# siyaoL1/Analytical-Database

Hardware: AMD Instinct MI355X
Metric: rows/sec scanned + HBM GB/s (% of roofline), 1B-row int32 select+sum (higher is better)
Workload: dtype int32; 1 GPU; 1B-row single int32 column, range select + sum; rows_per_gpu=1000000000, low=250000000, high=260000000, parallelism=single GPU

## Files before the change

### analytical-database_amd/csrc/mq_kernels.hip

```cpp

#include <hip/hip_runtime.h>

#include <atomic>
#include <condition_variable>
#include <mutex>
#include <thread>
#include <vector>
#include <climits>
#include <cstdarg>
#include <cstdint>
#include <cstdio>
#include <cstdlib>
#include <cstring>

#include <cerrno>
#include <pthread.h>
#include <sched.h>
#include <sys/mman.h>

#ifndef MADV_POPULATE_WRITE
#define MADV_POPULATE_WRITE 23
#endif

#include "mq_common.h"
#include "mq_device.h"
#include "mq_scan_common.h"

__device__ int mq_writelane(int src, int lane, int old) __asm("llvm.amdgcn.writelane.i32");

namespace {

using namespace mqi;

__device__ __forceinline__ void store_agent(unsigned long long* p, unsigned long long v) {
    __hip_atomic_store(p, v, __ATOMIC_RELAXED, __HIP_MEMORY_SCOPE_AGENT);
}
__device__ __forceinline__ unsigned long long load_agent(const unsigned long long* p) {
    return __hip_atomic_load(const_cast<unsigned long long*>(p), __ATOMIC_RELAXED,
                             __HIP_MEMORY_SCOPE_AGENT);
}

template <bool WT = false>
__device__ __forceinline__ void block_store_partial(unsigned long long cnt, long long sum, int mn,
                                                    int mx, Partial* __restrict__ part) {
    __shared__ Partial sp[kWaves];
    const int lane = threadIdx.x & 63, wave = threadIdx.x >> 6;
    cnt = wave_sum_u64(cnt);
    sum = wave_sum_i64(sum);
    mn = wave_min(mn);
    mx = wave_max(mx);
    if (lane == 0) sp[wave] = Partial{cnt, sum, mn, mx, 0ull};
    __syncthreads();
    if (threadIdx.x == 0) {
        Partial r = sp[0];
#pragma unroll
        for (int w = 1; w < kWaves; w++) {
            r.count += sp[w].count;
            r.sum += sp[w].sum;
            r.mn = min(r.mn, sp[w].mn);
            r.mx = max(r.mx, sp[w].mx);
        }
        if constexpr (WT) {
            unsigned long long* w = reinterpret_cast<unsigned long long*>(part + blockIdx.x);
            store_agent(w + 0, r.count);
            store_agent(w + 1, (unsigned long long)r.sum);
            store_agent(w + 2, (unsigned long long)(uint32_t)r.mn | ((unsigned long long)(uint32_t)r.mx << 32));
        } else {
            part[blockIdx.x] = r;
        }
    }
}

constexpr int kArriveStride = 1024;
constexpr size_t kArriveBytes = 9 * kArriveStride * sizeof(unsigned int);

__device__ __forceinline__ bool block_arrive_last(uint32_t nblocks, unsigned int* ctr) {
    __shared__ int s_last;
    if (threadIdx.x == 0) {
        const uint32_t shard = blockIdx.x & 7u;
        const uint32_t shard_n = (nblocks - shard + 7u) / 8u;
        __builtin_amdgcn_s_waitcnt(0x0F70);
        int last = 0;
        if (__hip_atomic_fetch_add(ctr + shard * kArriveStride, 1u, __ATOMIC_RELAXED,
                                   __HIP_MEMORY_SCOPE_AGENT) == shard_n - 1u) {
            const uint32_t nshards = nblocks < 8u ? nblocks : 8u;
            last = __hip_atomic_fetch_add(ctr + 8 * kArriveStride, 1u, __ATOMIC_RELAXED,
                                          __HIP_MEMORY_SCOPE_AGENT) == nshards - 1u;
        }
        if (last) {
#pragma unroll
            for (int i = 0; i < 9; i++)
                __hip_atomic_store(ctr + i * kArriveStride, 0u, __ATOMIC_RELAXED,
                                   __HIP_MEMORY_SCOPE_AGENT);
        }
        s_last = last;
    }
    __syncthreads();
    return s_last != 0;
}

__device__ __forceinline__ void block_combine(const Partial* __restrict__ part, uint32_t nparts,
                                              mq_agg* __restrict__ out) {
    unsigned long long cnt = 0;
    long long sum = 0;
    int mn = INT_MAX, mx = INT_MIN;
    for (uint32_t base = 0; base < nparts; base += 8 * blockDim.x) {
        unsigned long long c[8], sm[8], m[8];
#pragma unroll
        for (int j = 0; j < 8; j++) {
            const uint32_t i = base + j * blockDim.x + threadIdx.x;
            const unsigned long long* w =
                reinterpret_cast<const unsigned long long*>(part + (i < nparts ? i : nparts - 1));
            c[j] = load_agent(w + 0);
            sm[j] = load_agent(w + 1);
            m[j] = load_agent(w + 2);
        }
#pragma unroll
        for (int j = 0; j < 8; j++) {
            if (base + j * blockDim.x + threadIdx.x >= nparts) {
                c[j] = 0ull;
                sm[j] = 0ull;
                m[j] = 0x800000007FFFFFFFull;
            }
        }
#pragma unroll
        for (int j = 0; j < 8; j++) {
            cnt += c[j];
            sum += (long long)sm[j];
            mn = min(mn, (int)(uint32_t)m[j]);
            mx = max(mx, (int)(uint32_t)(m[j] >> 32));
        }
    }
    __shared__ Partial sc[kWaves];
    const int lane = threadIdx.x & 63, wave = threadIdx.x >> 6;
    cnt = wave_sum_u64(cnt);
    sum = wave_sum_i64(sum);
    mn = wave_min(mn);
    mx = wave_max(mx);
    if (lane == 0) sc[wave] = Partial{cnt, sum, mn, mx, 0ull};
    __syncthreads();
    if (threadIdx.x == 0) {
        Partial r = sc[0];
#pragma unroll
        for (int w = 1; w < kWaves; w++) {
            r.count += sc[w].count;
            r.sum += sc[w].sum;
            r.mn = min(r.mn, sc[w].mn);
            r.mx = max(r.mx, sc[w].mx);
        }
        out->count = r.count;
        out->sum = r.sum;
        out->min = r.mn;
        out->max = r.mx;
        out->_pad = 0;
    }
}

enum ScanMode { kSum = 0, kAgg = 1 };

template <int MODE>
struct ScanTraits {
    static constexpr int kUnrollM = MODE == kAgg ? 6 : kUnroll;
};

template <int MODE, bool VEC>
__global__ __launch_bounds__(kTPB, 8) void k_scan(const int* __restrict__ col, uint64_t n,
                                               uint64_t rows_per_block, Pred pred,
                                               Partial* __restrict__ part,
                                               mq_agg* __restrict__ out, unsigned int* __restrict__ arrive) {
    const uint64_t start = (uint64_t)blockIdx.x * rows_per_block;
    uint64_t end = start + rows_per_block;
    if (end > n) end = n;
    const int tid = threadIdx.x;
    const uint32_t lo = pred.lo, wm1 = pred.wm1;

    unsigned int cnt = 0;
    unsigned long long sumd = 0;
    uint32_t mind = 0xFFFFFFFFu;
    uint32_t maxr = 0xFFFFFFFFu;

    auto consume = [&](int4 v, uint64_t tile_row, bool full) {
        const uint64_t row = tile_row + (uint64_t)tid * 4;
        const uint32_t d0 = (uint32_t)v.x - lo, d1 = (uint32_t)v.y - lo, d2 = (uint32_t)v.z - lo,
                       d3 = (uint32_t)v.w - lo;
        bool p0 = d0 <= wm1, p1 = d1 <= wm1, p2 = d2 <= wm1, p3 = d3 <= wm1;
        if (!full) {
            p0 = p0 && (row + 0 < end);
            p1 = p1 && (row + 1 < end);
            p2 = p2 && (row + 2 < end);
            p3 = p3 && (row + 3 < end);
        }
        cnt += (unsigned)p0 + (unsigned)p1 + (unsigned)p2 + (unsigned)p3;
        sumd += (unsigned long long)(p0 ? d0 : 0u) + (unsigned long long)(p1 ? d1 : 0u) +
                (unsigned long long)(p2 ? d2 : 0u) + (unsigned long long)(p3 ? d3 : 0u);
        if constexpr (MODE == kAgg) {
            if (full) {
                mind = min(mind, min(min(d0, d1), min(d2, d3)));
                maxr = min(maxr, min(min(wm1 - d0, wm1 - d1), min(wm1 - d2, wm1 - d3)));
            } else {
                mind = min(mind, min(min(p0 ? d0 : ~0u, p1 ? d1 : ~0u), min(p2 ? d2 : ~0u, p3 ? d3 : ~0u)));
                maxr = min(maxr, min(min(p0 ? wm1 - d0 : ~0u, p1 ? wm1 - d1 : ~0u),
                                     min(p2 ? wm1 - d2 : ~0u, p3 ? wm1 - d3 : ~0u)));
            }
        }
    };

    constexpr int U = ScanTraits<MODE>::kUnrollM;
    uint64_t t = start;
    for (; t + (uint64_t)U * kTileRows <= end; t += (uint64_t)U * kTileRows) {
        int4 v[U];
#pragma unroll
        for (int u = 0; u < U; u++)
            v[u] = load4_nt<VEC>(col + t + (uint64_t)u * kTileRows + (uint64_t)tid * 4);
#pragma unroll
        for (int u = 0; u < U; u++) consume(v[u], t + (uint64_t)u * kTileRows, true);
    }
    for (; t < end; t += kTileRows) {
        const uint64_t row = t + (uint64_t)tid * 4;
        int4 v;
        if (row + 3 < end) {
            v = load4_nt<VEC>(col + row);
        } else {
            v.x = row + 0 < end ? col[row + 0] : 0;
            v.y = row + 1 < end ? col[row + 1] : 0;
            v.z = row + 2 < end ? col[row + 2] : 0;
            v.w = row + 3 < end ? col[row + 3] : 0;
        }
        consume(v, t, row + 3 < end);
    }
    const long long sum = (long long)sumd + (long long)cnt * (long long)(int32_t)lo;
    int mn = INT_MAX, mx = INT_MIN;
    if (MODE == kAgg && cnt) {
        mn = (int)(lo + mind);
        mx = (int)(lo + (wm1 - maxr));
    }
    if (out) {
        block_store_partial<true>(cnt, sum, mn, mx, part);
        if (block_arrive_last(gridDim.x, arrive)) block_combine(part, gridDim.x, out);
    } else {
        block_store_partial(cnt, sum, mn, mx, part);
    }
}

template <bool VEC>
__global__ __launch_bounds__(kTPB, 8) void k_stream_read(const int* __restrict__ col, uint64_t n,
                                                         uint64_t rows_per_block,
                                                         uint32_t* __restrict__ out) {
    const uint64_t start = (uint64_t)blockIdx.x * rows_per_block;
    uint64_t end = start + rows_per_block;
    if (end > n) end = n;
    const int tid = threadIdx.x;
    uint32_t x = 0;
    for (uint64_t t = start; t + 8ull * kTileRows <= end; t += 8ull * kTileRows) {
        int4 v[8];
#pragma unroll
        for (int u = 0; u < 8; u++)
            v[u] = load4_nt<VEC>(col + t + (uint64_t)u * kTileRows + (uint64_t)tid * 4);
#pragma unroll
        for (int u = 0; u < 8; u++) x ^= (uint32_t)(v[u].x ^ v[u].y ^ v[u].z ^ v[u].w);
    }
    x = (uint32_t)wave_sum_u64(x);
    if ((tid & 63) == 0) atomicXor(out + blockIdx.x, x);
}

__global__ __launch_bounds__(kTPB) void k_final(const Partial* __restrict__ part, uint32_t nparts,
                                                mq_agg* __restrict__ out) {
    unsigned long long cnt = 0;
    long long sum = 0;
    int mn = INT_MAX, mx = INT_MIN;
    for (uint32_t i = threadIdx.x; i < nparts; i += kTPB) {
        const Partial p = part[i];
        cnt += p.count;
        sum += p.sum;
        mn = min(mn, p.mn);
        mx = max(mx, p.mx);
    }
    __shared__ Partial sp[kWaves];
    const int lane = threadIdx.x & 63, wave = threadIdx.x >> 6;
    cnt = wave_sum_u64(cnt);
    sum = wave_sum_i64(sum);
    mn = wave_min(mn);
    mx = wave_max(mx);
    if (lane == 0) sp[wave] = Partial{cnt, sum, mn, mx, 0ull};
    __syncthreads();
    if (threadIdx.x == 0) {
        Partial r = sp[0];
        for (int w = 1; w < kWaves; w++) {
            r.count += sp[w].count;
            r.sum += sp[w].sum;
            r.mn = min(r.mn, sp[w].mn);
            r.mx = max(r.mx, sp[w].mx);
        }
        out->count = r.count;
        out->sum = r.sum;
        out->min = r.mn;
        out->max = r.mx;
        out->_pad = 0;
    }
}

constexpr int kStTiles = 8;
constexpr int kStGranule = 256 * kStTiles;
constexpr int kStBuf = 1024;
constexpr unsigned long long kStDone = 1ull << 63;

__device__ __forceinline__ uint32_t rank_lt(unsigned long long m, uint32_t acc) {
    return __builtin_amdgcn_mbcnt_hi((uint32_t)(m >> 32), __builtin_amdgcn_mbcnt_lo((uint32_t)m, acc));
}

struct StageState {
    uint32_t fill;
    uint32_t flushed;
    uint32_t nbm;
    uint64_t sw;
    bool bmode;
};

template <bool PAYLOAD, int BUF, bool FULL, int J>
__device__ __forceinline__ void stage_tile(StageState& st, int4 v, uint32_t t0, uint32_t E, uint32_t lo,
                                           uint32_t wm1, int32_t base, int lane, int* buf,
                                           const int* __restrict__ payload,
                                           unsigned long long* __restrict__ bm, int* __restrict__ spill,
                                           uint32_t r0, int& rlo, int& rhi) {
    const uint32_t row0 = t0 + (uint32_t)lane * 4;
    bool p0 = ((uint32_t)v.x - lo) <= wm1, p1 = ((uint32_t)v.y - lo) <= wm1,
         p2 = ((uint32_t)v.z - lo) <= wm1, p3 = ((uint32_t)v.w - lo) <= wm1;
    if (!FULL) {
        p0 = p0 && row0 + 0 < E;
        p1 = p1 && row0 + 1 < E;
        p2 = p2 && row0 + 2 < E;
        p3 = p3 && row0 + 3 < E;
    }
    const unsigned long long m0 = __ballot(p0), m1 = __ballot(p1), m2 = __ballot(p2),
                             m3 = __ballot(p3);
    const uint32_t c = __builtin_amdgcn_readfirstlane(
        (uint32_t)(__popcll(m0) + __popcll(m1) + __popcll(m2) + __popcll(m3)));
    if (!st.bmode) {
        if (c == 0) return;
        const uint32_t over = st.fill + c - st.flushed;
        const uint32_t need = __builtin_amdgcn_readfirstlane(
            over > (uint32_t)BUF ? ((over - (uint32_t)BUF + 63u) & ~63u) : 0u);
        if (st.flushed + need <= 8u * r0) {
            if (need) {
                __builtin_amdgcn_wave_barrier();
                for (uint32_t f = 0; f < need; f += 64u) {
                    const uint32_t i = st.flushed + f + (uint32_t)lane;
                    spill[i] = buf[i % (uint32_t)BUF];
                }
                st.flushed = __builtin_amdgcn_readfirstlane(st.flushed + need);
            }
            uint32_t k = rank_lt(m3, rank_lt(m2, rank_lt(m1, rank_lt(m0, st.fill))));
            if (p0) buf[(k++) % (uint32_t)BUF] = PAYLOAD ? payload[row0 + 0] : (int)(row0 + 0) + base;
            if (p1) buf[(k++) % (uint32_t)BUF] = PAYLOAD ? payload[row0 + 1] : (int)(row0 + 1) + base;
            if (p2) buf[(k++) % (uint32_t)BUF] = PAYLOAD ? payload[row0 + 2] : (int)(row0 + 2) + base;
            if (p3) buf[(k++) % (uint32_t)BUF] = PAYLOAD ? payload[row0 + 3] : (int)(row0 + 3) + base;
            st.fill = __builtin_amdgcn_readfirstlane(st.fill + c);
            return;
        }
        st.bmode = true;
        st.sw = t0;
    }
    if (J >= 0) {
        rlo = mq_writelane((int)m0, 4 * J + 0, rlo);
        rhi = mq_writelane((int)(m0 >> 32), 4 * J + 0, rhi);
        rlo = mq_writelane((int)m1, 4 * J + 1, rlo);
        rhi = mq_writelane((int)(m1 >> 32), 4 * J + 1, rhi);
        rlo = mq_writelane((int)m2, 4 * J + 2, rlo);
        rhi = mq_writelane((int)(m2 >> 32), 4 * J + 2, rhi);
        rlo = mq_writelane((int)m3, 4 * J + 3, rlo);
        rhi = mq_writelane((int)(m3 >> 32), 4 * J + 3, rhi);
    } else if (lane < 4) {
        bm[(uint64_t)(t0 >> 8) * 4 + (uint64_t)lane] = lane == 0 ? m0 : lane == 1 ? m1 : lane == 2 ? m2 : m3;
    }
    st.nbm = __builtin_amdgcn_readfirstlane(st.nbm + c);
}

__device__ __forceinline__ void load_pay4(int (&pv)[4], const int* __restrict__ payload, uint64_t r, uint64_t n,
                                          bool pal) {
    if (pal && r + 3 < n) {
        const int4 x = load4_nt<true>(payload + r);
        pv[0] = x.x;
        pv[1] = x.y;
        pv[2] = x.z;
        pv[3] = x.w;
    } else {
#pragma unroll
        for (int e = 0; e < 4; e++) pv[e] = payload[r + e < n ? r + e : n - 1];
    }
}

template <bool PAYLOAD, bool VEC, int BUF = kStBuf>
__global__ __launch_bounds__(kTPB, 8) void k_select_stage(
    const int* __restrict__ col, const int* __restrict__ payload, uint64_t n, uint64_t rw, Pred pred,
    unsigned long long* status, unsigned long long* __restrict__ bm, int* __restrict__ out,
    unsigned long long* __restrict__ d_count, unsigned int* err) {
    __shared__ __attribute__((aligned(16))) int s_buf[kWaves][BUF > 0 ? BUF : 1];
    __shared__ unsigned int s_cnt[kWaves];
    __shared__ unsigned long long s_red[kWaves];
    const int tid = threadIdx.x, lane = tid & 63;
    const int wave = __builtin_amdgcn_readfirstlane(tid >> 6);
    const uint32_t lo = pred.lo, wm1 = pred.wm1;
    const int32_t rbase = pred.base;
    const uint32_t b = blockIdx.x;
    uint64_t S = ((uint64_t)b * kWaves + (uint64_t)wave) * rw;
    if (S > n) S = n;
    uint64_t E = S + rw;
    if (E > n) E = n;
    StageState st{0u, 0u, 0u, E, false};
    int* spill = reinterpret_cast<int*>(bm + (S >> 8) * 4);
    int rlo = 0, rhi = 0;
    unsigned long long rec = 0;
    uint32_t rec_at = ~0u;
    const uint32_t S32 = (uint32_t)S, E32 = (uint32_t)E;
    uint32_t t = S32;
    for (; t + kStGranule <= E32; t += kStGranule) {
        const int* base = col + t;
        int4 v[kStTiles];
#pragma unroll
        for (int j = 0; j < kStTiles; j++) v[j] = load4_nt<VEC>(base + (uint32_t)(j * 256 + lane * 4));
        if (rec_at != ~0u && lane < 32) bm[(uint64_t)rec_at * 4 + (uint64_t)lane] = rec;
        rec_at = ~0u;
        const uint32_t r0 = (t - S32) >> 8;
#pragma unroll
        for (int j = 0; j < kStTiles; j++) {
            switch (j) {
#define MQ_ST(JJ) case JJ: stage_tile<PAYLOAD, BUF, true, JJ>(st, v[JJ], t + JJ * 256, E32, lo, wm1, rbase, lane, s_buf[wave], payload, bm, spill, r0, rlo, rhi); break;
                MQ_ST(0) MQ_ST(1) MQ_ST(2) MQ_ST(3) MQ_ST(4) MQ_ST(5) MQ_ST(6) MQ_ST(7)
#undef MQ_ST
            }
        }
        if (st.bmode) {
            rec = (unsigned long long)(uint32_t)rlo | ((unsigned long long)(uint32_t)rhi << 32);
            rec_at = t >> 8;
        }
    }
    if (rec_at != ~0u && lane < 32) bm[(uint64_t)rec_at * 4 + (uint64_t)lane] = rec;
    for (; t < E32; t += 256) {
        const uint32_t row = t + (uint32_t)lane * 4;
        int4 v;
        v.x = row + 0 < E32 ? col[row + 0] : 0;
        v.y = row + 1 < E32 ? col[row + 1] : 0;
        v.z = row + 2 < E32 ? col[row + 2] : 0;
        v.w = row + 3 < E32 ? col[row + 3] : 0;
        stage_tile<PAYLOAD, BUF, false, -1>(st, v, t, E32, lo, wm1, rbase, lane, s_buf[wave], payload, bm, spill,
                                            (t - S32) >> 8, rlo, rhi);
    }
    int* buf = s_buf[wave];
    const uint32_t fill = st.fill, nbm = st.nbm, flushed = st.flushed;
    const uint64_t sw = st.sw;

    const uint32_t mine = fill + nbm;
    if (lane == 0) s_cnt[wave] = mine;
    __syncthreads();
    unsigned long long blk = 0;
#pragma unroll
    for (int w = 0; w < kWaves; w++) blk += s_cnt[w];
    if (tid == 0) store_agent(&status[b], kStDone | blk);
    unsigned long long acc = 0;
    for (uint32_t i = tid; i < b; i += kTPB) {
        unsigned long long x;
        unsigned int spins = 0;
        while (!((x = load_agent(&status[i])) & kStDone)) {
            if (++spins > (1u << 26)) {
                atomicOr(err, 1u);
                x = kStDone;
                break;
            }
            __builtin_amdgcn_s_sleep(1);
        }
        acc += x & ~kStDone;
    }
    acc = wave_sum_u64(acc);
    if (lane == 0) s_red[wave] = acc;
    __syncthreads();
    unsigned long long D = 0;
#pragma unroll
    for (int w = 0; w < kWaves; w++) D += s_red[w];
    if (b == gridDim.x - 1 && tid == 0)
        *d_count = __hip_atomic_load(err, __ATOMIC_RELAXED, __HIP_MEMORY_SCOPE_AGENT) ? ~0ull : D + blk;
#pragma unroll
    for (int w = 0; w < kWaves; w++)
        if (w < wave) D += s_cnt[w];

    asm volatile("s_waitcnt vmcnt(0)" ::: "memory");
    for (uint32_t i0 = 0; i0 < flushed; i0 += 64u * 8u) {
        int x[8];
#pragma unroll
        for (int j = 0; j < 8; j++) {
            const uint32_t i = i0 + (uint32_t)j * 64u + (uint32_t)lane;
            x[j] = i < flushed ? spill[i] : 0;
        }
#pragma unroll
        for (int j = 0; j < 8; j++) {
            const uint32_t i = i0 + (uint32_t)j * 64u + (uint32_t)lane;
            if (i < flushed) out[D + i] = x[j];
        }
    }
    __builtin_amdgcn_wave_barrier();
    for (uint32_t i = flushed + (uint32_t)lane; i < fill; i += 64u) out[D + i] = buf[i % (uint32_t)BUF];
    if (sw >= E) return;
    unsigned long long o = D + fill;
    const uint64_t T1 = (E + 255) >> 8;
    const bool pal = PAYLOAD && ((reinterpret_cast<uintptr_t>(payload) & 15u) == 0);
    unsigned long long ob = o;
    uint32_t bfill = 0, bst = (uint32_t)(((uintptr_t)(out + ob) >> 2) & 3u);
    auto flush = [&]() {
        __builtin_amdgcn_wave_barrier();
        const uint32_t end = bst + bfill;
        int* base = out + ob - bst;
        for (uint32_t q = 4u * (uint32_t)lane; q < end; q += 256u) {
            if (q >= bst && q + 4u <= end) {
                *reinterpret_cast<int4*>(base + q) = *reinterpret_cast<const int4*>(buf + q);
            } else {
#pragma unroll
                for (uint32_t e = 0; e < 4; e++)
                    if (q + e >= bst && q + e < end) base[q + e] = buf[q + e];
            }
        }
        __builtin_amdgcn_wave_barrier();
        ob += bfill;
        bfill = 0;
        bst = (uint32_t)(((uintptr_t)(out + ob) >> 2) & 3u);
    };
    for (uint64_t tb = sw >> 8; tb < T1; tb += 64) {
        const uint64_t T = tb + (uint64_t)lane;
        unsigned long long w0 = 0, w1 = 0, w2 = 0, w3 = 0;
        if (T < T1) {
            const ulonglong2 a = reinterpret_cast<const ulonglong2*>(bm + T * 4)[0];
            const ulonglong2 c2 = reinterpret_cast<const ulonglong2*>(bm + T * 4)[1];
            w0 = a.x;
            w1 = a.y;
            w2 = c2.x;
            w3 = c2.y;
        }
        const unsigned int c = (unsigned int)(__popcll(w0) + __popcll(w1) + __popcll(w2) + __popcll(w3));
        unsigned int tot = c;
#pragma unroll
        for (int off = 32; off > 0; off >>= 1) tot += __shfl_xor(tot, off, 64);
        constexpr int kPf = PAYLOAD ? 4 : 1;
        for (int j0 = 0; j0 < 64; j0 += kPf) {
            int pv[kPf][4];
            if constexpr (PAYLOAD) {
#pragma unroll
                for (int jj = 0; jj < kPf; jj++) {
                    const uint64_t r = (tb + (uint64_t)(j0 + jj)) * 256 + 4 * (uint64_t)lane;
                    const bool any = __builtin_amdgcn_readlane((int)c, j0 + jj) != 0;
                    if (any) load_pay4(pv[jj], payload, r, n, pal);
                }
            }
#pragma unroll
            for (int jj = 0; jj < kPf; jj++) {
                const int j = j0 + jj;
                const uint32_t cj = (uint32_t)__builtin_amdgcn_readlane((int)c, j);
                if (cj == 0) continue;
                if (bst + bfill + cj > (uint32_t)BUF) flush();
                auto rl64 = [&](unsigned long long x) {
                    return (unsigned long long)(uint32_t)__builtin_amdgcn_readlane((int)(uint32_t)x, j) |
                           ((unsigned long long)(uint32_t)__builtin_amdgcn_readlane((int)(uint32_t)(x >> 32), j) << 32);
                };
                const unsigned long long x0 = rl64(w0), x1 = rl64(w1), x2 = rl64(w2), x3 = rl64(w3);
                const int rj = (int)((tb + (uint64_t)j) * 256 + 4 * (uint64_t)lane) + rbase;
                uint32_t k = bst + bfill + rank_lt(x3, rank_lt(x2, rank_lt(x1, rank_lt(x0, 0u))));
                if ((x0 >> lane) & 1ull) buf[k++] = PAYLOAD ? pv[jj][0] : rj + 0;
                if ((x1 >> lane) & 1ull) buf[k++] = PAYLOAD ? pv[jj][1] : rj + 1;
                if ((x2 >> lane) & 1ull) buf[k++] = PAYLOAD ? pv[jj][2] : rj + 2;
                if ((x3 >> lane) & 1ull) buf[k++] = PAYLOAD ? pv[jj][3] : rj + 3;
                bfill += cj;
            }
        }
        o += tot;
    }
    if (bfill) flush();
}

__global__ __launch_bounds__(kTPB) void k_hashset_lookup(const int32_t* __restrict__ table, int32_t size,
                                                         const int32_t* __restrict__ probe, uint64_t n,
                                                         uint8_t* __restrict__ found) {
    const uint64_t stride = (uint64_t)gridDim.x * kTPB;
    for (uint64_t i = (uint64_t)blockIdx.x * kTPB + threadIdx.x; i < n; i += stride) {
        const int32_t key = probe[i];
        int32_t idx = key % size;
        if (idx < 0) idx += size;
        int32_t v = table[idx];
        for (int32_t step = 1; v != 0 && v != key && step < size; step++) {
            idx = idx + 1 == size ? 0 : idx + 1;
            v = table[idx];
        }
        found[i] = (v != 0 && v == key) ? 1 : 0;
    }
}

template <bool VEC>
__device__ __forceinline__ void store4(int* __restrict__ p, int4 v) {
    if constexpr (VEC) {
        *reinterpret_cast<int4*>(p) = v;
    } else {
        p[0] = v.x;
        p[1] = v.y;
        p[2] = v.z;
        p[3] = v.w;
    }
}

template <bool VEC>
__global__ __launch_bounds__(kTPB) void k_fetch(const int* __restrict__ col,
                                                const int* __restrict__ pos, uint64_t k,
                                                int* __restrict__ out) {
    constexpr int kFetchU = 4;
    const uint64_t stride = (uint64_t)gridDim.x * kTPB;
    const uint64_t k4 = k / 4;
    uint64_t i0 = (uint64_t)blockIdx.x * kTPB + threadIdx.x;
    for (; i0 + (uint64_t)(kFetchU - 1) * stride < k4; i0 += stride * kFetchU) {
        int4 p[kFetchU], o[kFetchU];
#pragma unroll
        for (int u = 0; u < kFetchU; u++) p[u] = load4<VEC>(pos + (i0 + (uint64_t)u * stride) * 4);
#pragma unroll
        for (int u = 0; u < kFetchU; u++) {
            o[u].x = col[p[u].x];
            o[u].y = col[p[u].y];
            o[u].z = col[p[u].z];
            o[u].w = col[p[u].w];
        }
#pragma unroll
        for (int u = 0; u < kFetchU; u++) store4<VEC>(out + (i0 + (uint64_t)u * stride) * 4, o[u]);
    }
    for (; i0 < k4; i0 += stride) {
        const int4 p = load4<VEC>(pos + i0 * 4);
        store4<VEC>(out + i0 * 4, make_int4(col[p.x], col[p.y], col[p.z], col[p.w]));
    }
    if (blockIdx.x == 0 && threadIdx.x < (k & 3)) {
        const uint64_t i = k4 * 4 + threadIdx.x;
        out[i] = col[pos[i]];
    }
}

template <bool SUB, bool VEC>
__global__ __launch_bounds__(kTPB) void k_addsub(const int* __restrict__ a,
                                                 const int* __restrict__ b, uint64_t n,
                                                 int* __restrict__ out) {
    const uint64_t stride = (uint64_t)gridDim.x * kTPB;
    const uint64_t n4 = n / 4;
    for (uint64_t i = (uint64_t)blockIdx.x * kTPB + threadIdx.x; i < n4; i += stride) {
        const int4 x = load4<VEC>(a + i * 4), y = load4<VEC>(b + i * 4);
        int4 o;
        o.x = SUB ? (int)((uint32_t)x.x - (uint32_t)y.x) : (int)((uint32_t)x.x + (uint32_t)y.x);
        o.y = SUB ? (int)((uint32_t)x.y - (uint32_t)y.y) : (int)((uint32_t)x.y + (uint32_t)y.y);
        o.z = SUB ? (int)((uint32_t)x.z - (uint32_t)y.z) : (int)((uint32_t)x.z + (uint32_t)y.z);
        o.w = SUB ? (int)((uint32_t)x.w - (uint32_t)y.w) : (int)((uint32_t)x.w + (uint32_t)y.w);
        if constexpr (VEC) {
            *reinterpret_cast<int4*>(out + i * 4) = o;
        } else {
            out[i * 4 + 0] = o.x;
            out[i * 4 + 1] = o.y;
            out[i * 4 + 2] = o.z;
            out[i * 4 + 3] = o.w;
        }
    }
    if (blockIdx.x == 0 && threadIdx.x < (n & 3)) {
        const uint64_t i = n4 * 4 + threadIdx.x;
        out[i] = SUB ? (int)((uint32_t)a[i] - (uint32_t)b[i]) : (int)((uint32_t)a[i] + (uint32_t)b[i]);
    }
}

__device__ long long ref_binary_search(const int* __restrict__ a, long long size, int target) {
    long long left = 0, right = size - 1;
    while (left <= right) {
        const long long mid = (left + right) / 2;
        if (a[mid] == target) return mid;
        if (target < a[mid]) right = mid - 1;
        else left = mid + 1;
    }
    return right;
}

__global__ void k_index_bounds(const int* __restrict__ values, uint64_t n, int low, int high,
                               long long* __restrict__ run, unsigned long long* __restrict__ d_count) {
    if (threadIdx.x != 0 || blockIdx.x != 0) return;
    long long left = ref_binary_search(values, (long long)n, low);
    long long right = ref_binary_search(values, (long long)n, high);
    if (left < 0) {
        left = 0;
    } else {
        while (left > 0 && values[left] >= low) left--;
        if (values[left] != low) left++;
    }
    while (right > left && values[right] == high) right--;
    const long long k = right >= left ? right - left + 1 : 0;
    run[0] = left;
    run[1] = k;
    *d_count = (unsigned long long)k;
}

__global__ __launch_bounds__(kTPB) void k_index_copy(const uint64_t* __restrict__ positions,
                                                     const long long* __restrict__ run,
                                                     int* __restrict__ out) {
    const long long left = run[0], k = run[1];
    const long long stride = (long long)gridDim.x * kTPB;
    for (long long i = (long long)blockIdx.x * kTPB + threadIdx.x; i < k; i += stride)
        out[i] = (int)positions[left + i];
}

__device__ __forceinline__ uint64_t sm64(uint64_t x) {
    x += 0x9E3779B97F4A7C15ull;
    x = (x ^ (x >> 30)) * 0xBF58476D1CE4E5B9ull;
    x = (x ^ (x >> 27)) * 0x94D049BB133111EBull;
    return x ^ (x >> 31);
}

__device__ __forceinline__ uint32_t mix31(uint32_t x) {
    const uint32_t M = 0x7FFFFFFFu;
    x &= M;
    x = (uint32_t)(((uint64_t)x * 0x2545F491u) & M);
    x ^= x >> 15;
    x = (uint32_t)(((uint64_t)x * 0x4F6CDD1Du) & M);
    x ^= x >> 13;
    x = (uint32_t)(((uint64_t)x * 0x6A09E667u) & M);
    x ^= x >> 16;
    return x;
}

__global__ __launch_bounds__(kTPB) void k_gen_uniform(int* __restrict__ out, uint64_t n,
                                                      uint64_t base, uint64_t modulus) {
    const uint64_t stride = (uint64_t)gridDim.x * kTPB;
    for (uint64_t i = (uint64_t)blockIdx.x * kTPB + threadIdx.x; i < n; i += stride)
        out[i] = (int)(sm64(base + i) % modulus);
}

constexpr int kGBuf = 1024;

template <bool VEC>
__global__ __launch_bounds__(kTPB, 6) void k_scan_gather(const int* __restrict__ col,
                                                         const int* __restrict__ aux, uint64_t n,
                                                         uint64_t rows_per_block, Pred pred,
                                                         Partial* __restrict__ part,
                                                         mq_agg* __restrict__ out, unsigned int* __restrict__ arrive) {
    __shared__ uint32_t s_buf[kWaves][kGBuf];
    const uint64_t start = (uint64_t)blockIdx.x * rows_per_block;
    uint64_t end = start + rows_per_block;
    if (end > n) end = n;
    const int tid = threadIdx.x, lane = tid & 63, wave = tid >> 6;
    const uint32_t lo = pred.lo, wm1 = pred.wm1;
    uint32_t* buf = s_buf[wave];
    const int* auxb = aux + start;
    uint32_t fill = 0;
    unsigned long long cnt = 0;
    long long sumv = 0;
    int mnv = INT_MAX, mxv = INT_MIN;

    auto drain = [&]() {
        __builtin_amdgcn_wave_barrier();
        for (uint32_t i0 = 0; i0 < fill; i0 += 64u * 8u) {
            int x[8];
#pragma unroll
            for (int j = 0; j < 8; j++) {
                const uint32_t i = i0 + (uint32_t)j * 64u + (uint32_t)lane;
                x[j] = i < fill ? auxb[buf[i]] : 0;
            }
#pragma unroll
            for (int j = 0; j < 8; j++) {
                const uint32_t i = i0 + (uint32_t)j * 64u + (uint32_t)lane;
                if (i < fill) {
                    sumv += x[j];
                    mnv = min(mnv, x[j]);
                    mxv = max(mxv, x[j]);
                }
            }
        }
        __builtin_amdgcn_wave_barrier();
        fill = 0;
    };
    auto consume = [&](int4 v, uint64_t tile_row, bool full) {
        const uint64_t row = tile_row + (uint64_t)tid * 4;
        bool p0 = ((uint32_t)v.x - lo) <= wm1, p1 = ((uint32_t)v.y - lo) <= wm1,
             p2 = ((uint32_t)v.z - lo) <= wm1, p3 = ((uint32_t)v.w - lo) <= wm1;
        if (!full) {
            p0 = p0 && row + 0 < end;
            p1 = p1 && row + 1 < end;
            p2 = p2 && row + 2 < end;
            p3 = p3 && row + 3 < end;
        }
        const unsigned long long m0 = __ballot(p0), m1 = __ballot(p1), m2 = __ballot(p2),
                                 m3 = __ballot(p3);
        const uint32_t c = __builtin_amdgcn_readfirstlane(
            (uint32_t)(__popcll(m0) + __popcll(m1) + __popcll(m2) + __popcll(m3)));
        if (c == 0) return;
        cnt += c;
        if (fill + c > (uint32_t)kGBuf) drain();
        uint32_t k = rank_lt(m3, rank_lt(m2, rank_lt(m1, rank_lt(m0, fill))));
        const uint32_t r = (uint32_t)(row - start);
        if (p0) buf[k++] = r + 0;
        if (p1) buf[k++] = r + 1;
        if (p2) buf[k++] = r + 2;
        if (p3) buf[k++] = r + 3;
        fill = __builtin_amdgcn_readfirstlane(fill + c);
    };

    constexpr int U = 8;
    uint64_t t = start;
    for (; t + (uint64_t)U * kTileRows <= end; t += (uint64_t)U * kTileRows) {
        int4 v[U];
#pragma unroll
        for (int u = 0; u < U; u++)
            v[u] = load4_nt<VEC>(col + t + (uint64_t)u * kTileRows + (uint64_t)tid * 4);
#pragma unroll
        for (int u = 0; u < U; u++) consume(v[u], t + (uint64_t)u * kTileRows, true);
    }
    for (; t < end; t += kTileRows) {
        const uint64_t row = t + (uint64_t)tid * 4;
        int4 v;
        if (row + 3 < end) {
            v = load4_nt<VEC>(col + row);
        } else {
            v.x = row + 0 < end ? col[row + 0] : 0;
            v.y = row + 1 < end ? col[row + 1] : 0;
            v.z = row + 2 < end ? col[row + 2] : 0;
            v.w = row + 3 < end ? col[row + 3] : 0;
        }
        consume(v, t, row + 3 < end);
    }
    drain();
    const unsigned long long c_lane = lane == 0 ? cnt : 0ull;
    if (out) {
        block_store_partial<true>(c_lane, sumv, mnv, mxv, part);
        if (block_arrive_last(gridDim.x, arrive)) block_combine(part, gridDim.x, out);
    } else {
        block_store_partial(c_lane, sumv, mnv, mxv, part);
    }
}

__global__ __launch_bounds__(kTPB) void k_gen_join(int* __restrict__ out, uint64_t n, int kind) {
    const uint64_t stride = (uint64_t)gridDim.x * kTPB;
    const uint64_t mask = 2 * n - 1;
    for (uint64_t i = (uint64_t)blockIdx.x * kTPB + threadIdx.x; i < n; i += stride) {
        if (kind == 0) out[i] = (int)mix31((uint32_t)i);
        else if (kind == 1) out[i] = (int)mix31((uint32_t)(sm64((7ull << 40) | i) & mask));
        else if (kind == 2) out[i] = (int)mix31((uint32_t)(i % (n / 2 ? n / 2 : 1)));
        else out[i] = (int)mix31((uint32_t)(sm64((7ull << 40) | i) & (n - 1)));
    }
}

__global__ __launch_bounds__(kTPB) void k_copy16(uint4* __restrict__ dst, const uint4* __restrict__ src,
                                                 uint64_t n16, unsigned char* __restrict__ dtail,
                                                 const unsigned char* __restrict__ stail, uint32_t ntail) {
    const uint64_t stride = (uint64_t)gridDim.x * kTPB;
    uint64_t i = (uint64_t)blockIdx.x * kTPB + threadIdx.x;
    for (; i + 3 * stride < n16; i += 4 * stride) {
        const uint4 a = src[i], b = src[i + stride], c = src[i + 2 * stride], d = src[i + 3 * stride];
        dst[i] = a;
        dst[i + stride] = b;
        dst[i + 2 * stride] = c;
        dst[i + 3 * stride] = d;
    }
    for (; i < n16; i += stride) dst[i] = src[i];
    const uint32_t t = blockIdx.x * kTPB + threadIdx.x;
    if (t < ntail) dtail[t] = stail[t];
}

__global__ __launch_bounds__(kTPB) void k_copy1(unsigned char* __restrict__ dst, const unsigned char* __restrict__ src,
                                                uint64_t n) {
    const uint64_t stride = (uint64_t)gridDim.x * kTPB;
    for (uint64_t i = (uint64_t)blockIdx.x * kTPB + threadIdx.x; i < n; i += stride) dst[i] = src[i];
}

__global__ __launch_bounds__(kTPB) void k_iota(int* __restrict__ out, uint64_t n) {
    const uint64_t stride = (uint64_t)gridDim.x * kTPB;
    for (uint64_t i = (uint64_t)blockIdx.x * kTPB + threadIdx.x; i < n; i += stride) out[i] = (int)i;
}

}

namespace mqi {
thread_local char g_err[512] = "";

int set_err(int code, const char* fmt, ...) {
    va_list ap;
    va_start(ap, fmt);
    vsnprintf(g_err, sizeof(g_err), fmt, ap);
    va_end(ap);
    return code;
}

DevState g_dev[kMaxDev];

int current_device(int* dev) {
    int d = -1;
    hipError_t e = hipGetDevice(&d);
    if (e != hipSuccess || d < 0 || d >= kMaxDev)
        return set_err(MQ_ENODEV, "no HIP device: %s", hipGetErrorString(e));
    *dev = d;
    return MQ_OK;
}

int ensure_ready(DevState** out) {
    int d;
    int rc = current_device(&d);
    if (rc) return rc;
    DevState& s = g_dev[d];
    if (!s.ready) {
        hipDeviceProp_t prop;
        HIPCHK(hipGetDeviceProperties(&prop, d));
        if (strncmp(prop.gcnArchName, "gfx950", 6) != 0)
            return set_err(MQ_ENODEV, "device %d is %s, libmq is built for gfx950 only", d,
                           prop.gcnArchName);
        s.cus = prop.multiProcessorCount;
        s.ready = true;
    }
    *out = &s;
    return MQ_OK;
}

namespace {
struct PoolBlock {
    void* p;
    size_t bytes;
    int dev;
    bool busy;
    bool pending;
    hipEvent_t ev;
};
std::mutex g_pool_mu;
std::vector<PoolBlock> g_pool;

bool pool_in_flight(PoolBlock& b) {
    if (!b.pending) return false;
    if (hipEventQuery(b.ev) == hipErrorNotReady) return true;
    (void)hipGetLastError();
    b.pending = false;
    return false;
}

void pool_release_idle_locked() {
    for (size_t i = 0; i < g_pool.size();) {
        if (!g_pool[i].busy) {
            if (g_pool[i].pending) (void)hipEventSynchronize(g_pool[i].ev);
            if (g_pool[i].ev) (void)hipEventDestroy(g_pool[i].ev);
            (void)hipFree(g_pool[i].p);
            g_pool[i] = g_pool.back();
            g_pool.pop_back();
        } else {
            i++;
        }
    }
}
}

void* pool_alloc(size_t bytes) {
    if (bytes == 0) bytes = 16;
    int dev = 0;
    (void)hipGetDevice(&dev);
    std::unique_lock<std::mutex> lk(g_pool_mu);
    PoolBlock *best = nullptr, *wait = nullptr;
    for (auto& b : g_pool)
        if (!b.busy && b.dev == dev && b.bytes >= bytes && b.bytes / 2 <= bytes) {
            PoolBlock*& slot = pool_in_flight(b) ? wait : best;
            if (!slot || b.bytes < slot->bytes) slot = &b;
        }
    if (best) {
        best->busy = true;
        return best->p;
    }
    void* p = nullptr;
    if (hipMalloc(&p, bytes) != hipSuccess) {
        (void)hipGetLastError();
        if (wait) {
            wait->busy = true;
            void* q = wait->p;
            hipEvent_t ev = wait->ev;
            wait->pending = false;
            lk.unlock();
            (void)hipEventSynchronize(ev);
            return q;
        }
        pool_release_idle_locked();
        if (hipMalloc(&p, bytes) != hipSuccess) {
            (void)hipGetLastError();
            return nullptr;
        }
    }
    g_pool.push_back(PoolBlock{p, bytes, dev, true, false, nullptr});
    return p;
}

void pool_free(void* p) {
    if (!p) return;
    std::lock_guard<std::mutex> lk(g_pool_mu);
    for (auto& b : g_pool)
        if (b.p == p) {
            b.busy = false;
            return;
        }
    (void)hipFree(p);
}

void pool_free_on(void* p, hipStream_t st) {
    if (!p) return;
    int dev = -1;
    (void)hipGetDevice(&dev);
    std::unique_lock<std::mutex> lk(g_pool_mu);
    for (auto& b : g_pool)
        if (b.p == p) {
            bool ok = b.dev == dev;
            if (ok && !b.ev) ok = hipEventCreateWithFlags(&b.ev, hipEventDisableTiming) == hipSuccess;
            if (ok) ok = hipEventRecord(b.ev, st) == hipSuccess;
            if (!ok) {
                (void)hipGetLastError();
                lk.unlock();
                (void)hipStreamSynchronize(st);
                pool_free(p);
                return;
            }
            b.pending = true;
            b.busy = false;
            return;
        }
    lk.unlock();
    (void)hipStreamSynchronize(st);
    (void)hipFree(p);
}

uint32_t stream_grid(const DevState* s, uint64_t work_items) {
    uint64_t g = (work_items + kTPB - 1) / kTPB;
    const uint64_t cap = (uint64_t)s->cus * 8;
    if (g > cap) g = cap;
    return (uint32_t)(g == 0 ? 1 : g);
}

uint32_t resident_grid(const DevState* s, uint64_t work_items, const void* fn) {
    const uint32_t g = stream_grid(s, work_items);
    const uint64_t cap = (uint64_t)s->cus * (uint64_t)blocks_per_cu(fn);
    return cap && g > cap ? (uint32_t)cap : g;
}

bool make_pred(int has_low, int32_t low, int has_high, int32_t high, Pred* p) {
    const int64_t lo = has_low ? (int64_t)low : (int64_t)INT32_MIN;
    const int64_t hi = has_high ? (int64_t)high : (int64_t)INT32_MAX + 1;
    const int64_t width = hi - lo;
    if (width <= 0) return false;
    p->lo = (uint32_t)lo;
    p->wm1 = (uint32_t)(width - 1);
    p->base = 0;
    return true;
}

int blocks_per_cu(const void* fn, size_t dyn_lds) {
    struct Entry {
        int dev;
        const void* fn;
        size_t dyn;
        int occ;
    };
    static Entry cache[64];
    static int ncache = 0;
    static std::mutex mu;
    int dev = 0;
    if (hipGetDevice(&dev) != hipSuccess) dev = 0;
    std::lock_guard<std::mutex> lk(mu);
    for (int i = 0; i < ncache; i++)
        if (cache[i].dev == dev && cache[i].fn == fn && cache[i].dyn == dyn_lds) return cache[i].occ;
    int occ = 0;
    if (hipOccupancyMaxActiveBlocksPerMultiprocessor(&occ, fn, kTPB, dyn_lds) != hipSuccess || occ < 1)
        occ = 1;
    if (ncache < 64) cache[ncache++] = Entry{dev, fn, dyn_lds, occ};
    return occ;
}

void geometry(const DevState* s, uint64_t n, const void* fn, uint32_t* blocks, uint64_t* rpb,
              uint64_t granule, size_t dyn_lds, int bpc_cap) {
    int bpc = blocks_per_cu(fn, dyn_lds);
    if (bpc_cap > 0 && bpc > bpc_cap) bpc = bpc_cap;
    uint64_t gmax = (uint64_t)s->cus * (uint64_t)bpc;
    if (gmax > kMaxBlocks) gmax = kMaxBlocks;
    const uint64_t tiles = (n + granule - 1) / granule;
    uint64_t g = tiles < gmax ? tiles : gmax;
    if (g == 0) g = 1;
    const uint64_t tiles_per_block = (tiles + g - 1) / g;
    *rpb = (tiles_per_block == 0 ? 1 : tiles_per_block) * granule;
    g = (n + *rpb - 1) / *rpb;
    *blocks = (uint32_t)(g == 0 ? 1 : g);
}

size_t partial_bytes() { return (size_t)kMaxBlocks * sizeof(Partial); }
}

namespace {
using namespace mqi;

template <int MODE>
const void* scan_fn(bool vec) {
    return vec ? reinterpret_cast<const void*>(&k_scan<MODE, true>)
               : reinterpret_cast<const void*>(&k_scan<MODE, false>);
}

struct ArriveEntry {
    int dev;
    hipStream_t st;
    std::thread::id th;
    unsigned int* ctr;
};
std::mutex g_arrive_mu;
std::vector<ArriveEntry> g_arrive;

int stream_device(hipStream_t st, int* dev) {
    if (st != nullptr && st != hipStreamPerThread && hipStreamGetDevice(st, dev) == hipSuccess) return 0;
    return hipGetDevice(dev) == hipSuccess ? 0 : -1;
}

unsigned int* arrive_counters(hipStream_t st) {
    int dev = 0;
    if (stream_device(st, &dev)) return nullptr;
    const std::thread::id th = st == hipStreamPerThread ? std::this_thread::get_id() : std::thread::id();
    std::lock_guard<std::mutex> lk(g_arrive_mu);
    for (const ArriveEntry& e : g_arrive)
        if (e.dev == dev && e.st == st && e.th == th) return e.ctr;
    int cur = dev;
    (void)hipGetDevice(&cur);
    if (cur != dev && hipSetDevice(dev) != hipSuccess) return nullptr;
    void* p = nullptr;
    const bool ok = hipMalloc(&p, kArriveBytes) == hipSuccess;
    if (ok && hipMemsetAsync(p, 0, kArriveBytes, st) != hipSuccess) {
        (void)hipFree(p);
        p = nullptr;
    }
    if (cur != dev) (void)hipSetDevice(cur);
    if (!p) return nullptr;
    g_arrive.push_back(ArriveEntry{dev, st, th, static_cast<unsigned int*>(p)});
    return static_cast<unsigned int*>(p);
}
// ... 932 lines not shown
```

Before: 1689 billion rows/s.

## Fold block partials into sharded atomic accumulators instead of partial array combine

Each block now atomically adds its count and sum (and atomic-maxes the biased min/max) into one of 32 sharded accumulator slots, then does the two-level arrival counting. The last arriving block reads the 32 shards with one wave, resets them with exchanges, and writes the result. This replaces writing a per-block Partial array and having the last block reread all of it, which shrinks the tail of the single-pass scan. In exchange, every block issues more atomics, and the min/max encoding is more complex.

```diff
diff --git a/analytical-database_amd/csrc/mq_kernels.hip b/analytical-database_amd/csrc/mq_kernels.hip
--- a/analytical-database_amd/csrc/mq_kernels.hip
+++ b/analytical-database_amd/csrc/mq_kernels.hip
@@ -40,7 +40,6 @@
                              __HIP_MEMORY_SCOPE_AGENT);
 }
 
-template <bool WT = false>
 __device__ __forceinline__ void block_store_partial(unsigned long long cnt, long long sum, int mn,
                                                     int mx, Partial* __restrict__ part) {
     __shared__ Partial sp[kWaves];
@@ -60,98 +59,93 @@
             r.mn = min(r.mn, sp[w].mn);
             r.mx = max(r.mx, sp[w].mx);
         }
-        if constexpr (WT) {
-            unsigned long long* w = reinterpret_cast<unsigned long long*>(part + blockIdx.x);
-            store_agent(w + 0, r.count);
-            store_agent(w + 1, (unsigned long long)r.sum);
-            store_agent(w + 2, (unsigned long long)(uint32_t)r.mn | ((unsigned long long)(uint32_t)r.mx << 32));
-        } else {
-            part[blockIdx.x] = r;
-        }
-    }
-}
-
-constexpr int kArriveStride = 1024;
-constexpr size_t kArriveBytes = 9 * kArriveStride * sizeof(unsigned int);
-
-__device__ __forceinline__ bool block_arrive_last(uint32_t nblocks, unsigned int* ctr) {
-    __shared__ int s_last;
-    if (threadIdx.x == 0) {
-        const uint32_t shard = blockIdx.x & 7u;
-        const uint32_t shard_n = (nblocks - shard + 7u) / 8u;
-        __builtin_amdgcn_s_waitcnt(0x0F70);
-        int last = 0;
-        if (__hip_atomic_fetch_add(ctr + shard * kArriveStride, 1u, __ATOMIC_RELAXED,
-                                   __HIP_MEMORY_SCOPE_AGENT) == shard_n - 1u) {
-            const uint32_t nshards = nblocks < 8u ? nblocks : 8u;
-            last = __hip_atomic_fetch_add(ctr + 8 * kArriveStride, 1u, __ATOMIC_RELAXED,
-                                          __HIP_MEMORY_SCOPE_AGENT) == nshards - 1u;
-        }
-        if (last) {
-#pragma unroll
-            for (int i = 0; i < 9; i++)
-                __hip_atomic_store(ctr + i * kArriveStride, 0u, __ATOMIC_RELAXED,
-                                   __HIP_MEMORY_SCOPE_AGENT);
-        }
-        s_last = last;
-    }
-    __syncthreads();
-    return s_last != 0;
-}
-
-__device__ __forceinline__ void block_combine(const Partial* __restrict__ part, uint32_t nparts,
-                                              mq_agg* __restrict__ out) {
-    unsigned long long cnt = 0;
-    long long sum = 0;
-    int mn = INT_MAX, mx = INT_MIN;
-    for (uint32_t base = 0; base < nparts; base += 8 * blockDim.x) {
-        unsigned long long c[8], sm[8], m[8];
-#pragma unroll
-        for (int j = 0; j < 8; j++) {
-            const uint32_t i = base + j * blockDim.x + threadIdx.x;
-            const unsigned long long* w =
-                reinterpret_cast<const unsigned long long*>(part + (i < nparts ? i : nparts - 1));
-            c[j] = load_agent(w + 0);
-            sm[j] = load_agent(w + 1);
-            m[j] = load_agent(w + 2);
-        }
-#pragma unroll
-        for (int j = 0; j < 8; j++) {
-            if (base + j * blockDim.x + threadIdx.x >= nparts) {
-                c[j] = 0ull;
-                sm[j] = 0ull;
-                m[j] = 0x800000007FFFFFFFull;
-            }
-        }
-#pragma unroll
-        for (int j = 0; j < 8; j++) {
-            cnt += c[j];
-            sum += (long long)sm[j];
-            mn = min(mn, (int)(uint32_t)m[j]);
-            mx = max(mx, (int)(uint32_t)(m[j] >> 32));
-        }
-    }
-    __shared__ Partial sc[kWaves];
+        part[blockIdx.x] = r;
+    }
+}
+
+constexpr int kArriveShards = 32;
+constexpr int kArriveWords = 5;
+constexpr int kArriveStride = 32;
+constexpr size_t kArriveBytes = (size_t)(1 + kArriveShards * kArriveWords) * kArriveStride * sizeof(unsigned int);
+static_assert(kArriveShards <= 64, "the last arriver reads one shard per lane of one wave");
+
+__device__ __forceinline__ unsigned int* arrive_word(unsigned int* ctr, uint32_t shard, int k) {
+    return ctr + (size_t)(1u + shard * kArriveWords + (uint32_t)k) * kArriveStride;
+}
+
+template <bool MINMAX>
+__device__ __forceinline__ void block_fold_arrive(unsigned long long cnt, long long sum, int mn,
+                                                  int mx, uint32_t nblocks, unsigned int* ctr,
+                                                  mq_agg* __restrict__ out) {
+    __shared__ Partial sp[kWaves];
     const int lane = threadIdx.x & 63, wave = threadIdx.x >> 6;
     cnt = wave_sum_u64(cnt);
     sum = wave_sum_i64(sum);
     mn = wave_min(mn);
     mx = wave_max(mx);
-    if (lane == 0) sc[wave] = Partial{cnt, sum, mn, mx, 0ull};
+    if (lane == 0) sp[wave] = Partial{cnt, sum, mn, mx, 0ull};
     __syncthreads();
-    if (threadIdx.x == 0) {
-        Partial r = sc[0];
-#pragma unroll
-        for (int w = 1; w < kWaves; w++) {
-            r.count += sc[w].count;
-            r.sum += sc[w].sum;
-            r.mn = min(r.mn, sc[w].mn);
-            r.mx = max(r.mx, sc[w].mx);
-        }
-        out->count = r.count;
-        out->sum = r.sum;
-        out->min = r.mn;
-        out->max = r.mx;
+    if (wave != 0) return;
+    Partial r = sp[0];
+#pragma unroll
+    for (int w = 1; w < kWaves; w++) {
+        r.count += sp[w].count;
+        r.sum += sp[w].sum;
+        r.mn = min(r.mn, sp[w].mn);
+        r.mx = max(r.mx, sp[w].mx);
+    }
+    const uint32_t shard = blockIdx.x % (uint32_t)kArriveShards;
+    if (r.count != 0ull && lane < (MINMAX ? 4 : 2)) {
+        unsigned int* w = arrive_word(ctr, shard, 1 + lane);
+        unsigned long long seen;
+        if (lane < 2)
+            seen = __hip_atomic_fetch_add(reinterpret_cast<unsigned long long*>(w),
+                                          lane == 0 ? r.count : (unsigned long long)r.sum,
+                                          __ATOMIC_RELAXED, __HIP_MEMORY_SCOPE_AGENT);
+        else
+            seen = __hip_atomic_fetch_max(w, lane == 2 ? (uint32_t)INT_MAX - (uint32_t)r.mn
+                                                       : (uint32_t)r.mx - (uint32_t)INT_MIN,
+                                          __ATOMIC_RELAXED, __HIP_MEMORY_SCOPE_AGENT);
+        asm volatile("" ::"v"(seen) : "memory");
+    }
+    int last = 0;
+    if (lane == 0) {
+        __builtin_amdgcn_s_waitcnt(0x0F70);
+        const uint32_t shard_n = (nblocks - shard + (uint32_t)kArriveShards - 1u) / (uint32_t)kArriveShards;
+        if (__hip_atomic_fetch_add(arrive_word(ctr, shard, 0), 1u, __ATOMIC_RELAXED,
+                                   __HIP_MEMORY_SCOPE_AGENT) == shard_n - 1u) {
+            const uint32_t nshards = nblocks < (uint32_t)kArriveShards ? nblocks : (uint32_t)kArriveShards;
+            last = __hip_atomic_fetch_add(ctr, 1u, __ATOMIC_RELAXED, __HIP_MEMORY_SCOPE_AGENT) ==
+                   nshards - 1u;
+        }
+    }
+    if (!__shfl(last, 0, 64)) return;
+    const uint32_t nshards = nblocks < (uint32_t)kArriveShards ? nblocks : (uint32_t)kArriveShards;
+    unsigned long long c = 0ull, s = 0ull;
+    uint32_t dmin = 0u, dmax = 0u;
+    if ((uint32_t)lane < nshards) {
+        c = __hip_atomic_exchange(reinterpret_cast<unsigned long long*>(arrive_word(ctr, lane, 1)), 0ull,
+                                  __ATOMIC_RELAXED, __HIP_MEMORY_SCOPE_AGENT);
+        s = __hip_atomic_exchange(reinterpret_cast<unsigned long long*>(arrive_word(ctr, lane, 2)), 0ull,
+                                  __ATOMIC_RELAXED, __HIP_MEMORY_SCOPE_AGENT);
+        if constexpr (MINMAX) {
+            dmin = __hip_atomic_exchange(arrive_word(ctr, lane, 3), 0u, __ATOMIC_RELAXED,
+                                         __HIP_MEMORY_SCOPE_AGENT);
+            dmax = __hip_atomic_exchange(arrive_word(ctr, lane, 4), 0u, __ATOMIC_RELAXED,
+                                         __HIP_MEMORY_SCOPE_AGENT);
+        }
+        __hip_atomic_store(arrive_word(ctr, lane, 0), 0u, __ATOMIC_RELAXED, __HIP_MEMORY_SCOPE_AGENT);
+    }
+    if (lane == 0) __hip_atomic_store(ctr, 0u, __ATOMIC_RELAXED, __HIP_MEMORY_SCOPE_AGENT);
+    c = wave_sum_u64(c);
+    s = wave_sum_u64(s);
+    const int rmn = wave_min((int)((uint32_t)INT_MAX - dmin));
+    const int rmx = wave_max((int)(dmax + (uint32_t)INT_MIN));
+    if (lane == 0) {
+        out->count = c;
+        out->sum = (long long)s;
+        out->min = rmn;
+        out->max = rmx;
         out->_pad = 0;
     }
 }
@@ -235,8 +229,7 @@
         mx = (int)(lo + (wm1 - maxr));
     }
     if (out) {
-        block_store_partial<true>(cnt, sum, mn, mx, part);
-        if (block_arrive_last(gridDim.x, arrive)) block_combine(part, gridDim.x, out);
+        block_fold_arrive<MODE == kAgg>(cnt, sum, mn, mx, gridDim.x, arrive, out);
     } else {
         block_store_partial(cnt, sum, mn, mx, part);
     }
@@ -821,8 +814,7 @@
     drain();
     const unsigned long long c_lane = lane == 0 ? cnt : 0ull;
     if (out) {
-        block_store_partial<true>(c_lane, sumv, mnv, mxv, part);
-        if (block_arrive_last(gridDim.x, arrive)) block_combine(part, gridDim.x, out);
+        block_fold_arrive<true>(c_lane, sumv, mnv, mxv, gridDim.x, arrive, out);
     } else {
         block_store_partial(c_lane, sumv, mnv, mxv, part);
     }
```

After: 1698 billion rows/s, median of 6. About the same (+0.5%).
